# roncapat/UNIGE-TASI-path-planners

Measured on AMD Instinct MI355X. Metric: grid cells updated/sec (full plan + 100 replans), 4096^2 map, higher is better.
Workload: dtype f32

## Files before the change

### unige-tasi-path-planners_amd/csrc/ufm_control.h

```cpp
#pragma once

__global__ void k_fill(float *p, size_t n, float v) {
    for (size_t i = (size_t)blockIdx.x * blockDim.x + threadIdx.x; i < n; i += (size_t)gridDim.x * blockDim.x) p[i] = v;
}

__device__ __forceinline__ void patch_apply(const DevParams &P, int m, const uint8_t *patch, uint8_t *pmask, int x, int y, int w, int h, int e) {
    if (e >= w * h) return;
    const int i = e / w, j = e - i * w;
    uint8_t *cm = P.cost + (size_t)m * P.cstride;
    const size_t ci = (size_t)(x + i) * P.W + (y + j);
    const uint8_t nv = patch[e];
    const uint8_t ch = cm[ci] != nv;
    pmask[e] = ch;
    if (ch) { cm[ci] = nv; cost_window_store(P, m, x + i, y + j, nv); }
}
__global__ void k_patch_apply(DevParams P, int m, const uint8_t *patch, uint8_t *pmask, int x, int y, int w, int h) {
    patch_apply(P, m, patch, pmask, x, y, w, h, blockIdx.x * blockDim.x + threadIdx.x);
}
template <bool NODES>
__device__ __forceinline__ void patch_seed(const DevParams &P, int m, const uint8_t *pmask, int x, int y, int w, int h, int e) {
    const int ew = NODES ? w + 1 : w, eh = NODES ? h + 1 : h;
    bool hit = false;
    int gt = -1;
    if (e < ew * eh) {
        const int i = e / ew, j = e - i * ew;
        bool ch;
// ... 336 lines not shown
        const int cx = x - 1 + (q >> 1), cy = y - 1 + (q & 1);
        const float c = cst(cx, cy), g1 = h ? val(x, y + dy) : val(x + dx, y), g2 = val(x + dx, y + dy);
        float r; int dep;
        if constexpr (ALGO == UFM_ALGO_SG) { CellSG k; k.set(c); r = tri_sg(g1, g2, k); dep = dep_sg(g1, g2, k); }
        else {
            const float bb = h ? cst(x - 1 + (1 - (q >> 1)), cy) : cst(cx, y - 1 + (1 - (q & 1)));
            CellFD k{c, c * c, c * SQRT2F}; TriFD t; t.set(c, bb);
            r = tri_fd(g1, g2, k, t); dep = dep_fd(g1, g2, k, t);
        }
        if (r > g || r != r) {
            const float B = P.dyn->focused ? start_bound(P, m) : INFINITY;
            if (g + tile_heuristic(P, m, x / T, y / T) < B || B == INFINITY) ++n_bad; else ++n_parked;
        }
        else if (r < g) ++n_low;
        else if (dep != (b & 3)) ++n_dep;
    }
    if (n_val) atomicAdd(&out[0], n_val);
    if (n_none) atomicAdd(&out[1], n_none);
    if (n_bad) atomicAdd(&out[2], n_bad);
    if (n_dep) atomicAdd(&out[3], n_dep);
    if (n_low) atomicAdd(&out[4], n_low);
    if (n_parked) atomicAdd(&out[5], n_parked);
}
__global__ void k_cost_stats(const uint8_t *cm, size_t n, int thr, unsigned long long *out) {
    unsigned long long s = 0, c = 0;
    for (size_t i = (size_t)blockIdx.x * blockDim.x + threadIdx.x; i < n; i += (size_t)gridDim.x * blockDim.x) {
        const int v = cm[i];
        if (v < thr) { s += v; ++c; }
    }
    for (int o = 32; o > 0; o >>= 1) { s += __shfl_down(s, o); c += __shfl_down(c, o); }
    if ((threadIdx.x & 63) == 0) { atomicAdd(&out[0], s); atomicAdd(&out[1], c); }
}
__device__ __forceinline__ void finalize_tiles(const DevParams &P) {
    const int n = P.ctr->tcount;
    for (int i = blockIdx.x; i < n; i += gridDim.x) {
        const int gt = P.tlist[i];
        const size_t gidx = (size_t)gt * TT + threadIdx.x;
        const int diff = (threadIdx.x < T * T) && (P.fresh[gt] ? (P.G[gidx] != INFINITY) : (P.G[gidx] != P.Gprev[gidx]));
        const int c = __syncthreads_count(diff);
        if (threadIdx.x == 0) {
            if (c) atomicAdd(&P.ctr->expanded, (unsigned long long)c);
            P.touched[gt] = 0;
        }
    }
}
__global__ __launch_bounds__(256) void k_finalize(DevParams P, int only_if_done) {
    if (only_if_done && !P.ctr->done) return;
    const int n = P.ctr->tcount;
    const int lane = threadIdx.x & 63;
    const int wave = (blockIdx.x * blockDim.x + threadIdx.x) >> 6, nwaves = (gridDim.x * blockDim.x) >> 6;
    unsigned long long total = 0;
    for (int i = wave; i < n; i += nwaves) {
        const int gt = P.tlist[i];
        const float *g = P.G + (size_t)gt * TT, *g0 = P.Gprev + (size_t)gt * TT;
        int c = 0;
        if (P.fresh[gt]) {
#pragma unroll
            for (int e = lane; e < TT; e += 64) c += (g[e] != INFINITY) ? 1 : 0;
        } else {
#pragma unroll
            for (int e = lane; e < TT; e += 64) c += (g[e] != g0[e]) ? 1 : 0;
        }
        total += (unsigned long long)c;
        if (lane == 0) P.touched[gt] = 0;
    }
    for (int o = 32; o > 0; o >>= 1) total += __shfl_down(total, o);
    if (lane == 0 && total) atomicAdd(&P.ctr->expanded, total);
}
template <int ALGO>
__device__ void tile_bp(const DevParams &P, int gt, int thr, float *Gs, float *Cs) {
    constexpr int CROWS = is_dfm<ALGO> ? T : T + 1, COFF = is_dfm<ALGO> ? 0 : 1, CN = CROWS * CROWS;
    const int tid = threadIdx.x, w = tid >> 6, lane = tid & 63, q = lane & 3, nd = lane >> 2;
    const int m = gt / P.NTm, t = gt - m * P.NTm, tx = t / P.TY, ty = t - tx * P.TY, x0 = tx * T, y0 = ty * T;
    const float *Gt = P.G + (size_t)gt * TT, *ring = P.ring + (size_t)gt * RING;
    const uint8_t *ct = P.costT + (size_t)gt * CTS;
    for (int e = tid; e < TT; e += 256) Gs[(e / T + 1) * GP + e % T + 1] = Gt[e];
    for (int ht = tid; ht < 4 * T + 4; ht += 256) {
        int hr, hc;
        if (ht < T) { hr = -1; hc = ht; }
        else if (ht < 2 * T) { hr = T; hc = ht - T; }
        else if (ht < 3 * T) { hr = ht - 2 * T; hc = -1; }
        else if (ht < 4 * T) { hr = ht - 3 * T; hc = T; }
        else { hr = (ht & 2) ? T : -1; hc = (ht & 1) ? T : -1; }
        Gs[(hr + 1) * GP + hc + 1] = ring[ht];
    }
    for (int e = tid; e < CN; e += 256) {
        const int cr = e / CROWS, cc = e - cr * CROWS, cx = x0 + cr - COFF, cy = y0 + cc - COFF, c = ct[e];
        Cs[cr * CP + cc] = (cx < 0 || cy < 0 || cx >= P.L || cy >= P.W || c >= thr) ? INFINITY : (float)c;
    }
    __syncthreads();
    const int goal_x = P.goal[2 * m], goal_y = P.goal[2 * m + 1];
    for (int p = w; p < PT * PT; p += 4) {
        const int lx = (p / PT) * 4 + (nd >> 2), ly = (p % PT) * 4 + (nd & 3);
        QuadConsts<ALGO> C;
        C.load(Cs, lx, ly, q);
        const LaneEval le = eval_quad_w<ALGO>(Gs + (lx + 1) * GP + ly + 1, q, C);
        const float nv = quad_min(le.r);
        const int bq = quad_min_int(bp_byte<ALGO>(le, q, C, le.r == nv)), b = bp_of_key<ALGO>(bq);
        if (q == 0) P.bp[(size_t)gt * TT + lx * T + ly] = (uint8_t)((x0 + lx == goal_x && y0 + ly == goal_y) ? BP_NONE : b);
    }
    __syncthreads();
}
template <int ALGO>
__global__ __launch_bounds__(256) void k_finalize_bp(DevParams P, int only_if_done) {
    __shared__ float Gs[(T + 2) * GP];
    __shared__ float Cs[(T + 1) * CP];
    if (only_if_done && !P.ctr->done) return;
    const int n = P.ctr->tcount, thr = P.dyn->thr;
    for (int i = blockIdx.x; i < n; i += gridDim.x) tile_bp<ALGO>(P, P.tlist[i], thr, Gs, Cs);
}
__global__ __launch_bounds__(T * T) void k_replan_end(DevParams P, int kr, int kl, float margin,
                                                      DevCounters *host, unsigned int *flag, unsigned int seq) {
    __shared__ int s_m, s_done, s_last;
    kr = launch_index(P, Q_RAISE, kr);
    kl = launch_index(P, Q_LOWER, kl);
    if (seq == 0) seq = P.ctr->pubseq;
    const int done = replan_check(P, kr, kl, margin, blockIdx.x == 0, s_m, s_done);
    if (done) finalize_tiles(P);
    __threadfence();
    __syncthreads();
    if (threadIdx.x == 0) s_last = (atomicAdd(&P.ctr->fin_blocks, 1) == (int)gridDim.x - 1);
    __syncthreads();
    if (!s_last) return;
    __threadfence();
    if (threadIdx.x == 0) P.ctr->fin_blocks = 0;
    const int *src = reinterpret_cast<const int *>(P.ctr);
    int *dst = reinterpret_cast<int *>(host);
    for (int i = threadIdx.x; i < (int)(sizeof(DevCounters) / sizeof(int)); i += blockDim.x)
        dst[i] = __hip_atomic_load(&src[i], __ATOMIC_RELAXED, __HIP_MEMORY_SCOPE_AGENT);
    __threadfence_system();
    __syncthreads();
    if (threadIdx.x == 0) __hip_atomic_store(flag, seq, __ATOMIC_RELEASE, __HIP_MEMORY_SCOPE_SYSTEM);
// ... 41 lines not shown
```

### unige-tasi-path-planners_amd/csrc/ufm_defs.h

```cpp
#pragma once


#ifndef UFM_TILE
#define UFM_TILE 16
#endif
constexpr int T = UFM_TILE;
static_assert(T == 32 || T == 16, "tile edge must be 32 or 16");
constexpr int GP = T + 8;
constexpr int CP = T + 2;
constexpr int PT = T / 4;
constexpr int PR = PT / 4;
constexpr int PPW = PR * PR;
constexpr int NTHR = 1024;
#ifndef UFM_RELAX_WAVES
#define UFM_RELAX_WAVES 4
#endif
#ifndef UFM_CAUSAL_FILTER
#define UFM_CAUSAL_FILTER 1
#endif
#ifndef UFM_STEP_FILTER
#define UFM_STEP_FILTER 1
#endif
#ifndef UFM_DFM1_LAX_VISITS
#define UFM_DFM1_LAX_VISITS 64
// ... 115 lines not shown
    int npark[2];
    int nready[2];
    int rcursor[2];
    int nshort[2];
    int last_work[2];
    int fin_blocks;
    int kbase[2];
    unsigned int pubseq;
    int tcount;
    int scount;
    unsigned long long expanded;
    unsigned long long tile_visits;
    unsigned long long tile_iters;
    unsigned long long elem_evals;
    int qmin[2];
    float rbound;
    int done;
    unsigned int updated;
    int done_fail;
    unsigned long long raise_visits;
    int own_stops;
    int own_abort;
    unsigned long long own_vis0, own_vis1;
};

struct DevDyn {
    float hm;
    int thr;
    int focused;
    int pad;
};

struct DevParams {
    float *G;
    float *Gprev;
    uint8_t *bp;
    float *ring;
    float *seen;
    uint8_t *cost;
    uint8_t *costT;
    int *goal;
    int *cand;
    int *ready;
    int *hint;
    int *rank;
    int *park;
// ... 177 lines not shown
```

### unige-tasi-path-planners_amd/csrc/ufm_engine.hip

```cpp
#include <hip/hip_runtime.h>
#include <hip/hip_ext.h>

#include <chrono>
#include <climits>
#include <cmath>
#include <cstddef>
#include <cstdio>
#include <cstdlib>
#include <cstring>
#include <new>
#include <type_traits>
#include <thread>
#include <vector>

#include "../../include/ufm.h"

namespace {

#include "ufm_defs.h"
#include "ufm_ops.h"
#include "ufm_relax.h"
#include "ufm_control.h"

#include "ufm_region.h"
// ... 50 lines not shown
int ufm_debug_tiles(unsigned int *out, int n) {
    if (n > TILE_DIAG_MAX) n = TILE_DIAG_MAX;
    for (int r = 0; r < 5; ++r)
        if (hipMemcpyFromSymbol(out + (size_t)r * n, HIP_SYMBOL(g_tile), sizeof(unsigned int) * n, sizeof(unsigned int) * (size_t)r * TILE_DIAG_MAX) != hipSuccess) return UFM_ERR_HIP_BASE;
    return n;
}
int ufm_debug_wtrace(unsigned long long *out, unsigned int *counts) {
    if (hipMemcpyFromSymbol(out, HIP_SYMBOL(g_wtrace), sizeof(unsigned long long) * 16 * 256 * 2) != hipSuccess) return UFM_ERR_HIP_BASE;
    if (hipMemcpyFromSymbol(counts, HIP_SYMBOL(g_nw), sizeof(unsigned int) * 16) != hipSuccess) return UFM_ERR_HIP_BASE;
    unsigned int z[16] = {};
    hipMemcpyToSymbol(HIP_SYMBOL(g_nw), z, sizeof(z));
    return UFM_OK;
}
int ufm_debug_tdiag(unsigned long long *out, int reset) {
    if (out && hipMemcpyFromSymbol(out, HIP_SYMBOL(g_tdiag), sizeof(unsigned long long) * 64) != hipSuccess) return UFM_ERR_HIP_BASE;
    if (reset) { unsigned long long z[64] = {}; if (hipMemcpyToSymbol(HIP_SYMBOL(g_tdiag), z, sizeof(z)) != hipSuccess) return UFM_ERR_HIP_BASE; }
    return UFM_OK;
}
#endif
int ufm_debug_lmax(ufm_t *p, int32_t *out, int n) {
    if (!p || !p->e->allocated || n > LMAX) return UFM_ERR_INVALID;
    hipStreamSynchronize(p->e->stream);
    return hipMemcpy(out, p->e->P.lmax, sizeof(int) * n, hipMemcpyDeviceToHost) == hipSuccess ? UFM_OK : UFM_ERR_HIP_BASE;
}
int ufm_debug_set_tile_order(ufm_t *p, const float *a, int n) {
    if (!p || !p->e->allocated || !a || n != p->e->P.NT) return UFM_ERR_INVALID;
    hipStreamSynchronize(p->e->stream);
    if (hipMemcpy(p->e->P.dag_a, a, sizeof(float) * (size_t)n, hipMemcpyHostToDevice) != hipSuccess) return UFM_ERR_HIP_BASE;
    p->e->dag_have = true;
    return UFM_OK;
}
int ufm_tile_edge(void) { return T; }
#ifdef UFM_STRICT_FENCES
const char *ufm_version(void) { return "ufm-gfx950 0.1 (block-FIM, strict-fence checking build)"; }
#else
const char *ufm_version(void) { return T == 32 ? "ufm-gfx950 0.1 (block-FIM, tile 32)" : "ufm-gfx950 0.1 (block-FIM, tile 16)"; }
#endif

int ufm_create(ufm_t **out, int algo, int opt_lvl, int use_heuristic, int device_id) {
    if (!out) return UFM_ERR_INVALID;
    Engine *e = nullptr;
    int rc = engine_create(&e, 1, algo, opt_lvl, use_heuristic, device_id);
    if (rc != UFM_OK) return rc;
    *out = new ufm_planner{e};
    return UFM_OK;
}
// ... 298 lines not shown
```

### unige-tasi-path-planners_amd/csrc/ufm_host.h

```cpp
#pragma once

#define HIPCHK(expr)                                                      \
    do {                                                                  \
        hipError_t _e = (expr);                                           \
        if (_e != hipSuccess) return UFM_ERR_HIP_BASE - (int)_e;          \
    } while (0)

struct PatchRect { int m, x, y, w, h; };

#include "ufm_path.h"

struct MapState {
    bool initialize_search = true;
    bool goal_set = false;
    bool new_goal = false;
    bool new_start = false;
    bool have_map = false;
    bool start_set = false;
    float start_x = 0, start_y = 0, goal_x = 0, goal_y = 0;
    int goal_ex = 0, goal_ey = 0;
    bool goal_elem_valid = false;
};

struct Engine {
// ... 26 lines not shown
    int owned_waves = 0;
    int dag_mode = 0;
    bool dag_have = false;
    float dag_kappa = 0.5f;
    int dag_patience = 16;
    bool dfm_follow_info = false;
    bool use_region = true;
    int region_ahead = 2;
    int region_tiles = 6;
    int region_sweeps = 4096;
    int region_debug = 0;
    float region_band = 1.5f;
    uint32_t region_runs = 0, region_done = 0;
    uint32_t region_cont = 0, region_cont_done = 0;
    int cont_raise = 4, cont_lower = 8;
    int batch_margin = 1;
    float raise_margin = 0.25f;
    ReplanJob *h_job = nullptr;
    struct GraphSig { DevParams P; float band, delta; int max_iters, grid, follow; };
    GraphSig graph_sig{};
    std::vector<std::pair<int, hipGraphExec_t>> graphs;
    int relax_kernel(int mode, int k_arg, float rbound, int grid);
    void finalize_bp(int only_if_done) {
        if (algo == UFM_ALGO_FD) k_finalize_bp<UFM_ALGO_FD><<<2048, 256, 0, stream>>>(P, only_if_done);
        else if (algo == UFM_ALGO_SG) k_finalize_bp<UFM_ALGO_SG><<<2048, 256, 0, stream>>>(P, only_if_done);
        else if (opt_lvl >= 1) k_finalize_bp<ALGO_DFM1><<<2048, 256, 0, stream>>>(P, only_if_done);
    }
    int tail_grid = 96;
    int replan_graph(int nr, int nl, float band, hipGraphExec_t *out);
    void drop_graphs() { for (auto &g : graphs) hipGraphExecDestroy(g.second); graphs.clear(); }
    int *h_scratch = nullptr;
    int *d_scratch = nullptr;
    uint8_t *d_patch = nullptr;
    size_t d_patch_cap = 0;
    uint8_t *h_patch = nullptr;
    float *d_field = nullptr;
    size_t d_field_cap = 0;
    int32_t *d_info = nullptr;
    size_t d_info_cap = 0;
    uint8_t *d_pmask = nullptr;
    size_t d_pmask_cap = 0;
    PathJob *d_jobs = nullptr, *h_jobs = nullptr;
    float *d_path = nullptr, *h_path = nullptr;
    size_t path_cap = 0;
    std::vector<MapState> maps;
    std::vector<PatchRect> pending;
    std::vector<PatchRect> region_rects;
    int iter[2] = {0, 0};
    bool focused = true;
// ... 53 lines not shown
    int flush_lazy();
    int ensure_pmask(size_t n);
    bool region_fits(const int (*rects)[5], int nrect, int m, int *tx0, int *ntx, int *ty0, int *nty) const;
    bool track = false;
    float *trk_g = nullptr;
    uint8_t *trk_key = nullptr;
    void *trk_rec = nullptr;
    size_t trk_cap = 0;
    hipEvent_t trk_ev[2] = {nullptr, nullptr};
    float trk_scan_ms = 0.0f;
    int track_alloc();
    int track_reset(int m);
    int track_records(size_t cap);
    void track_free();
    bool lazy_region_ok() const;
};

void Engine::release() {
    if (!allocated) return;
    if (stream) hipStreamSynchronize(stream);
    track_free();
    drop_graphs();
    deferred.clear();
    std::memset(&graph_sig, 0, sizeof(graph_sig));
    void *ptrs[] = {P.G, P.Gprev, P.bp, P.ring, P.seen, P.cost, P.costT, P.goal, P.cand, P.ready, P.hint, P.rank, P.park, P.pflag, P.pprio,
                    P.queued, P.prio, P.start, P.bnd, P.dyn, P.spos, P.touched, P.fresh, P.tlist, P.sflag, P.slist, P.slist2,
                    P.mark, P.num_updated, P.consume, P.lmax, P.own_prio, P.own_lock, P.own_min, P.dag_a, P.dag_thr, P.dag_left, P.ctr, d_scratch};
    for (void *q : ptrs) if (q) hipFree(q);
    P = DevParams{};
    d_scratch = nullptr;
    allocated = false;
}

int Engine::alloc(int width, int length) {
    release();
    W = width; L = length;
    const bool nodes = algo != UFM_ALGO_DFM;
    P.W = W; P.L = L;
    P.EX = nodes ? L + 1 : L;
    P.EY = nodes ? W + 1 : W;
    P.TX = (P.EX + T - 1) / T;
    P.TY = (P.EY + T - 1) / T;
    if ((long long)P.TX * P.TY * nmaps > (long long)INT32_MAX / 4 || (long long)P.EX * P.EY > INT32_MAX) return UFM_ERR_NOMEM;
    P.NTm = P.TX * P.TY;
    P.nmaps = nmaps;
    P.NT = P.NTm * nmaps;
// ... 52 lines not shown
    dmalloc(P.dag_left, sizeof(int) * own_words());
    dmalloc(P.ctr, sizeof(DevCounters));
    dmalloc(d_scratch, sizeof(int) * (4 * nmaps + 16));
    if (rc != UFM_OK) { release(); return rc; }
    rc = [&]() -> int {
        HIPCHK(hipMemsetAsync(P.cand, 0, sizeof(int) * 6 * P.NT, stream));
        HIPCHK(hipMemsetAsync(P.park, 0, sizeof(int) * 4 * P.NT, stream));
        HIPCHK(hipMemsetAsync(P.ready, 0, sizeof(int) * P.NT, stream));
        HIPCHK(hipMemsetAsync(P.tlist, 0, sizeof(int) * P.NT, stream));
        HIPCHK(hipMemsetAsync(P.slist, 0, sizeof(int) * P.NT, stream));
        HIPCHK(hipMemsetAsync(P.slist2, 0, sizeof(int) * P.NT, stream));
        HIPCHK(hipMemsetAsync(P.rank, 0, sizeof(int) * P.NT, stream));
        HIPCHK(hipMemsetAsync(P.hint, 0, sizeof(int) * P.NT, stream));
        HIPCHK(hipMemsetAsync(P.spos, 0, sizeof(float) * 2 * nmaps, stream));
        HIPCHK(hipMemsetAsync(P.start, 0xFF, sizeof(int) * 4 * nmaps, stream));
        HIPCHK(hipMemsetAsync(P.ctr, 0, sizeof(DevCounters), stream));
        { int rq = reset_queues(); if (rq != UFM_OK) return rq; }
        HIPCHK(hipMemsetAsync(P.touched, 0, sizeof(int) * P.NT, stream));
        HIPCHK(hipMemsetAsync(P.fresh, 0, (size_t)P.NT, stream));
        HIPCHK(hipMemsetAsync(P.sflag, 0, sizeof(int) * P.NT, stream));
        HIPCHK(hipMemsetAsync(P.mark, 0, P.mstride * nmaps, stream));
        HIPCHK(hipMemsetAsync(P.num_updated, 0, sizeof(unsigned int) * nmaps, stream));
        HIPCHK(hipMemsetAsync(P.goal, 0xFF, sizeof(int) * 2 * nmaps, stream));
        k_fill<<<1024, 256, 0, stream>>>(P.G, P.gstride * nmaps, INFINITY);
        k_fill<<<1024, 256, 0, stream>>>(P.Gprev, P.gstride * nmaps, INFINITY);
        HIPCHK(hipMemsetAsync(P.bp, BP_NONE, P.gstride * nmaps, stream));
        k_fill<<<1024, 256, 0, stream>>>(P.ring, (size_t)P.NT * RING, INFINITY);
        dyn_dev = DevDyn{heur ? heuristic_multiplier : 0.0f, thr_uchar, focused ? 1 : 0, 0};
        k_set_dyn<<<1, 1, 0, stream>>>(P.dyn, dyn_dev);
        HIPCHK(hipGetLastError());
        return UFM_OK;
    }();
    if (rc != UFM_OK) { release(); return rc; }
    if (track) { rc = track_alloc(); if (rc != UFM_OK) { release(); return rc; } }
    pending.clear();
    for (auto &ms : maps) { ms.have_map = false; ms.initialize_search = true; }
    return UFM_OK;
}

int Engine::reset_queues() {
    HIPCHK(hipMemsetAsync(P.queued, 0, sizeof(int) * 4 * P.NT, stream));
    HIPCHK(hipMemsetAsync(P.prio, 0xFF, sizeof(unsigned long long) * 4 * P.NT, stream));
    HIPCHK(hipMemsetAsync(P.pflag, 0, sizeof(int) * 2 * P.NT, stream));
    k_fill<<<64, 256, 0, stream>>>(reinterpret_cast<float *>(P.pprio), (size_t)2 * P.NT, INFINITY);
    k_fill<<<64, 256, 0, stream>>>(reinterpret_cast<float *>(P.own_prio), own_words(), INFINITY);
    HIPCHK(hipMemsetAsync(P.own_lock, 0, sizeof(int) * own_words(), stream));
    k_fill<<<2, 256, 0, stream>>>(reinterpret_cast<float *>(P.own_min), (size_t)OWN_NW, INFINITY);
    static_assert(offsetof(DevCounters, cnt) == 0, "queue state leads the counter block");
    HIPCHK(hipMemsetAsync(P.ctr, 0, offsetof(DevCounters, kbase), stream));
    k_fill<<<1, 64, 0, stream>>>(reinterpret_cast<float *>(&P.ctr->lmin[0][0]), (size_t)6, INFINITY);
    last_active = 1;
    iter[0] = iter[1] = 0;
    return UFM_OK;
}
int Engine::read_bounds(float *bmax) {
    k_start_bound<<<(nmaps + 63) / 64, 64, 0, stream>>>(P);
    HIPCHK(hipMemcpyAsync(h_bnd, P.bnd, sizeof(float) * nmaps, hipMemcpyDeviceToHost, stream));
    HIPCHK(hipStreamSynchronize(stream));
    float b = 0.0f;
    for (int m = 0; m < nmaps; ++m) b = std::fmax(b, h_bnd[m]);
    *bmax = b;
    return UFM_OK;
}

__global__ void k_publish(const DevCounters *src, DevCounters *dst, unsigned int *flag, unsigned int seq) {
    const int *s = reinterpret_cast<const int *>(src);
    int *d = reinterpret_cast<int *>(dst);
    for (int i = threadIdx.x; i < (int)(sizeof(DevCounters) / sizeof(int)); i += blockDim.x) d[i] = s[i];
    __threadfence_system();
    __syncthreads();
    if (threadIdx.x == 0) __hip_atomic_store(flag, seq, __ATOMIC_RELEASE, __HIP_MEMORY_SCOPE_SYSTEM);
}
int Engine::fetch_counters() {
// ... 375 lines not shown
    }
    const DevDyn dyn_now{heur ? heuristic_multiplier : 0.0f, thr_uchar, focused ? 1 : 0, 0};
    bool dyn_pending = std::memcmp(&dyn_now, &dyn_dev, sizeof(DevDyn)) != 0;
    auto flush_dyn = [&]() {
        if (!dyn_pending) return;
        k_set_dyn<<<1, 1, 0, stream>>>(P.dyn, dyn_now);
        dyn_dev = dyn_now; dyn_pending = false;
    };

    int n_init = 0, n_upd = 0;
    int *consume = h_scratch, *init_tiles = h_scratch + nmaps, *goals = h_scratch + 2 * nmaps;
    {
        bool all_init = true;
        for (int m = 0; m < nmaps; ++m) all_init = all_init && (maps[m].initialize_search || maps[m].new_goal);
        if (all_init) { int rc = reset_queues(); if (rc != UFM_OK) return rc; }
    }
    for (int m = 0; m < nmaps; ++m) {
        MapState &ms = maps[m];
        consume[m] = 0;
        if (ms.initialize_search || ms.new_goal) {
            consume[m] = 1;
            goals[2 * m] = ms.goal_elem_valid ? ms.goal_ex : -1;
            goals[2 * m + 1] = ms.goal_elem_valid ? ms.goal_ey : -1;
            k_fill<<<1024, 256, 0, stream>>>(P.G + (size_t)m * P.gstride, P.gstride, INFINITY);
            HIPCHK(hipMemsetAsync(P.bp + (size_t)m * P.gstride, BP_NONE, P.gstride, stream));
            k_fill<<<256, 256, 0, stream>>>(P.ring + (size_t)m * P.NTm * RING, (size_t)P.NTm * RING, INFINITY);
            if (ms.goal_elem_valid) init_tiles[n_init++] = m * P.NTm + (ms.goal_ex / T) * P.TY + (ms.goal_ey / T);
            else ++n_init;
        } else if (ms.new_start) {
            ms.new_start = false;
            consume[m] = 1;
            ++n_upd;
        }
    }
    for (int m = 0; m < nmaps; ++m) {
        MapState &ms = maps[m];
        if (ms.initialize_search || ms.new_goal)
            HIPCHK(hipMemcpyAsync(P.goal + 2 * m, goals + 2 * m, 2 * sizeof(int), hipMemcpyHostToDevice, stream));
    }
    ReplanBegin rb{};
    bool fused = single && fuse_control && spin_wait && n_init == 0 && n_upd > 0 && !pending.empty() && pending.size() <= 4;
    if (fused)
        for (const PatchRect &r : pending) fused = fused && consume[r.m] && (r.w + 1) * (r.h + 1) <= 65 * 65;
    {
        int *st_el = h_scratch + 5 * nmaps + 4;
        float *sp = reinterpret_cast<float *>(h_scratch + 9 * nmaps + 8);
        for (int m = 0; m < nmaps; ++m) {
            const MapState &ms = maps[m];
            for (int i = 0; i < 4; ++i) st_el[4 * m + i] = -1;
            sp[2 * m] = sp[2 * m + 1] = 0.0f;
            if (!ms.start_set) continue;
            const int cx = (int)(start_cell_floor ? std::floor(ms.start_x) : std::roundf(ms.start_x)), cy = (int)(start_cell_floor ? std::floor(ms.start_y) : std::roundf(ms.start_y));
            sp[2 * m] = (algo == UFM_ALGO_DFM) ? (float)cx : ms.start_x;
            sp[2 * m + 1] = (algo == UFM_ALGO_DFM) ? (float)cy : ms.start_y;
            const int ncorner = (algo == UFM_ALGO_DFM) ? 1 : 4;
            for (int i = 0; i < ncorner; ++i) {
                const int ex = cx + (i & 1), ey = cy + (i >> 1);
// ... 291 lines not shown
                owned_left = h_ctr->cnt[Q_LOWER][iter[Q_LOWER] % 3];
            }
            int rc = owned_left == 0 ? UFM_OK : run_phase(MODE_LOWER, INFINITY, &ll, &st.kernel_ms, &st.timed_launches);
            if (rc != UFM_OK) return rc;
            st.launches += ll;
            bool again = false;
            if (focused && do_raise) {
                float bnew = 0.0f;
                rc = read_bounds(&bnew);
                if (rc != UFM_OK) return rc;
                k_queue_min<<<1, 1024, 0, stream>>>(P, Q_RAISE, iter[Q_RAISE]);
                rc = fetch_counters();
                if (rc != UFM_OK) return rc;
                float qm;
                std::memcpy(&qm, &h_ctr->qmin[Q_RAISE], sizeof(float));
                if (qm < bnew) { again = true; rbound = std::fmax(bnew, rbound) + band; }
            }
            const auto tc = std::chrono::steady_clock::now();
            u_acc += std::chrono::duration<double, std::milli>(tb - ta).count();
            p_acc += std::chrono::duration<double, std::milli>(tc - tb).count();
            if (!again) break;
        }
        const auto td = std::chrono::steady_clock::now();
        finalize_bp(0);
        k_finalize<<<2048, 256, 0, stream>>>(P, 0);
        { int rc = fetch_counters(); if (rc != UFM_OK) return rc; }
        st.expanded = h_ctr->expanded;
        st.tile_visits = h_ctr->tile_visits;
        st.tile_iters = h_ctr->tile_iters;
        st.elem_evals = h_ctr->elem_evals;
        st.raise_tile_visits = h_ctr->raise_visits;
        if (st.resident_launches) {
            st.resident_tile_visits = h_ctr->own_vis1 - h_ctr->own_vis0;
            st.resident_stops = (uint32_t)h_ctr->own_stops;
            if (own_timed) HIPCHK(hipEventElapsedTime(&st.resident_kernel_ms, own_ev[0], own_ev[1]));
        }
        if (profiling) {
            std::vector<int> lm(LMAX);
            HIPCHK(hipMemcpy(lm.data(), P.lmax, sizeof(int) * LMAX, hipMemcpyDeviceToHost));
            for (int v : lm) st.crit_sweeps += (uint64_t)v;
        }
        p_acc += std::chrono::duration<double, std::milli>(std::chrono::steady_clock::now() - td).count();
    } else if (fast_done) {
        st.expanded = h_ctr->expanded;
        st.tile_visits = h_ctr->tile_visits;
        st.tile_iters = h_ctr->tile_iters;
        st.elem_evals = h_ctr->elem_evals;
        st.raise_tile_visits = h_ctr->raise_visits;
        const double dt = std::chrono::duration<double, std::milli>(std::chrono::steady_clock::now() - t_seed).count();
        u_acc += 0.5 * dt;
        p_acc += 0.5 * dt;
    } else {
        HIPCHK(hipStreamSynchronize(stream));
    }
    for (int m = 0; m < nmaps; ++m) maps[m].new_goal = maps[m].initialize_search = false;
    st.updated = updated;
    st.queued_lower = (uint32_t)(h_ctr->cnt[Q_LOWER][iter[Q_LOWER] % 3] + h_ctr->npark[Q_LOWER]);
    st.queued_raise = (uint32_t)(h_ctr->cnt[Q_RAISE][iter[Q_RAISE] % 3] + h_ctr->npark[Q_RAISE]);
    st.graphs_instantiated = graphs_made;
    st.region_replans = region_runs; st.region_replans_done = region_done;
    st.u_ms = (float)u_acc;
    st.p_ms = (float)p_acc;
    last = st;
    if (out) *out = st;
// ... 80 lines not shown
    if (e->h_lazy) hipHostFree(e->h_lazy);
    e->drop_graphs();
    if (e->h_ctr) hipHostFree(e->h_ctr);
    for (int i = 0; i < 2; ++i) if (e->h_pipe_ctr[i]) hipHostFree(e->h_pipe_ctr[i]);
    if (e->h_job) hipHostFree(e->h_job);
    if (e->h_scratch) hipHostFree(e->h_scratch);
    if (e->h_bnd) hipHostFree(e->h_bnd);
    if (e->stream) hipStreamDestroy(e->stream);
    delete e;
    return UFM_OK;
}

int engine_set_map(Engine *e, int m, const uint8_t *src, bool on_device, int width, int length) {
    if (!e || !src || m < 0 || m >= e->nmaps || width <= 0 || length <= 0) return UFM_ERR_INVALID;
    HIPCHK(hipSetDevice(e->device));
    if (e->allocated) { int rc = e->flush_deferred(); if (rc != UFM_OK) return rc; }
    if (!e->allocated || width != e->W || length != e->L) {
        bool others = false;
        for (int k = 0; k < e->nmaps; ++k) if (k != m && e->maps[k].have_map) others = true;
        if (e->allocated && others) return UFM_ERR_INVALID;
        int rc = e->alloc(width, length);
        if (rc != UFM_OK) return rc;
    }
    HIPCHK(hipMemcpyAsync(e->P.cost + (size_t)m * e->P.cstride, src, (size_t)width * length,
                          on_device ? hipMemcpyDeviceToDevice : hipMemcpyHostToDevice, e->stream));
    k_cost_windows<<<2048, 256, 0, e->stream>>>(e->P, m);
    {
        unsigned long long *d_acc = reinterpret_cast<unsigned long long *>(e->d_scratch);
        HIPCHK(hipMemsetAsync(d_acc, 0, 2 * sizeof(unsigned long long), e->stream));
        k_cost_stats<<<512, 256, 0, e->stream>>>(e->P.cost + (size_t)m * e->P.cstride, (size_t)width * length, e->thr_uchar, d_acc);
        unsigned long long *h_acc = reinterpret_cast<unsigned long long *>(e->h_scratch);
        HIPCHK(hipMemcpyAsync(h_acc, d_acc, 2 * sizeof(unsigned long long), hipMemcpyDeviceToHost, e->stream));
        HIPCHK(hipStreamSynchronize(e->stream));
        if (h_acc[1] > 0) e->mean_cost = (float)((double)h_acc[0] / (double)h_acc[1]);
    }
    if (e->track) { int rc = e->track_reset(m); if (rc != UFM_OK) return rc; }
    e->maps[m].have_map = true;
    MapState &ms = e->maps[m];
    if (ms.goal_set) ms.goal_elem_valid = ms.goal_ex >= 0 && ms.goal_ey >= 0 && ms.goal_ex < e->P.EX && ms.goal_ey < e->P.EY;
    return UFM_OK;
}

int engine_patch(Engine *e, int m, const uint8_t *src, bool on_device, int x, int y, int w, int h) {
    if (!e || !src) return UFM_ERR_INVALID;
    HIPCHK(hipSetDevice(e->device));
    if (on_device) return e->patch(m, src, x, y, w, h, true);
    if (w <= 0 || h <= 0) return UFM_ERR_INVALID;
    {
        bool taken = false;
        const int rc = e->patch_lazy(m, src, x, y, w, h, &taken);
        if (rc != UFM_OK || taken) return rc;
    }
    const size_t n = (size_t)w * h;
// ... 164 lines not shown
```

Measured before the change: 566.5 million.

## Batch fills, fuse set_map stats with window build, wave-per-tile finalize

Replaces the many separate fill kernels and memsets with one table-driven fill kernel that writes 16-byte stores. Fuses the cost copy, the cost statistics and the tile window construction into a single k_set_map kernel. Fuses the finalize expanded-count into the backpointer kernel, which now assigns one wave per tile and uses wave-local LDS waits instead of block barriers. Also moves the lmax sum for profiling onto the device. These cut launch overhead and redundant passes over memory, at the cost of more complex code and more LDS per block.

```diff
diff --git a/unige-tasi-path-planners_amd/csrc/ufm_control.h b/unige-tasi-path-planners_amd/csrc/ufm_control.h
--- a/unige-tasi-path-planners_amd/csrc/ufm_control.h
+++ b/unige-tasi-path-planners_amd/csrc/ufm_control.h
@@ -2,6 +2,23 @@
 
 __global__ void k_fill(float *p, size_t n, float v) {
     for (size_t i = (size_t)blockIdx.x * blockDim.x + threadIdx.x; i < n; i += (size_t)gridDim.x * blockDim.x) p[i] = v;
+}
+
+constexpr int FILL_MAX = 24;
+struct FillTable { int n; struct { void *p; size_t bytes; unsigned int pat; } e[FILL_MAX]; };
+__global__ __launch_bounds__(256) void k_fill_table(FillTable t) {
+    const size_t gtid = (size_t)blockIdx.x * blockDim.x + threadIdx.x, gsz = (size_t)gridDim.x * blockDim.x;
+    for (int k = 0; k < t.n; ++k) {
+        unsigned int *w = static_cast<unsigned int *>(t.e[k].p);
+        const unsigned int pat = t.e[k].pat;
+        const size_t nw = t.e[k].bytes / 4;
+        const size_t lead = ((16 - (reinterpret_cast<uintptr_t>(w) & 15)) & 15) / 4, head = lead < nw ? lead : nw, nv = (nw - head) / 4, tail0 = head + nv * 4;
+        uint4 *v = reinterpret_cast<uint4 *>(w + head);
+        const uint4 pv = make_uint4(pat, pat, pat, pat);
+        for (size_t i = gtid; i < nv; i += gsz) v[i] = pv;
+        if (gtid < head) w[gtid] = pat;
+        if (gtid < nw - tail0) w[tail0 + gtid] = pat;
+    }
 }
 
 __device__ __forceinline__ void patch_apply(const DevParams &P, int m, const uint8_t *patch, uint8_t *pmask, int x, int y, int w, int h, int e) {
@@ -384,15 +401,90 @@
     if (n_low) atomicAdd(&out[4], n_low);
     if (n_parked) atomicAdd(&out[5], n_parked);
 }
-__global__ void k_cost_stats(const uint8_t *cm, size_t n, int thr, unsigned long long *out) {
-    unsigned long long s = 0, c = 0;
-    for (size_t i = (size_t)blockIdx.x * blockDim.x + threadIdx.x; i < n; i += (size_t)gridDim.x * blockDim.x) {
-        const int v = cm[i];
-        if (v < thr) { s += v; ++c; }
-    }
-    for (int o = 32; o > 0; o >>= 1) { s += __shfl_down(s, o); c += __shfl_down(c, o); }
-    if ((threadIdx.x & 63) == 0) { atomicAdd(&out[0], s); atomicAdd(&out[1], c); }
-}
+constexpr int SM_TILES = 16;
+constexpr int SM_CH = SM_TILES * T / 16;
+constexpr int SM_PITCH = SM_TILES * T + 16;
+template <bool CELLS>
+__global__ __launch_bounds__(256) void k_set_map(DevParams P, int m, const uint8_t *src, int thr, unsigned long long *out) {
+    constexpr int CROWS = CELLS ? T : T + 1, OFF = CELLS ? 0 : 1, CN = CROWS * CROWS, NCH = (CN + 15) / 16;
+    static_assert(NCH * 16 <= CTS, "the 16-byte stores stay inside a window record");
+    __shared__ __attribute__((aligned(16))) uint8_t s[(T + 1) * SM_PITCH];
+    const int nstrips = (P.TY + SM_TILES - 1) / SM_TILES;
+    const int tx = blockIdx.x / nstrips, ty0 = (blockIdx.x - tx * nstrips) * SM_TILES, x0 = tx * T, y0 = ty0 * T;
+    uint8_t *cm = P.cost + (size_t)m * P.cstride;
+    const bool copy = src != cm;
+    const bool vec = ((reinterpret_cast<uintptr_t>(src) | reinterpret_cast<uintptr_t>(cm) | (uintptr_t)P.W) & 15) == 0;
+    unsigned int sum = 0, cnt = 0;
+    for (int task = threadIdx.x; task < (T + 1) * (SM_CH + 1); task += blockDim.x) {
+        const int r = task / (SM_CH + 1), k = task - r * (SM_CH + 1) - 1;
+        const int cx = x0 - 1 + r;
+        const bool rowin = cx >= 0 && cx < P.L && !(CELLS && r == 0), own = r > 0;
+        if (k < 0) {
+            const int cy = y0 - 1;
+            s[r * SM_PITCH + 15] = (rowin && !CELLS && cy >= 0 && cy < P.W) ? src[(size_t)cx * P.W + cy] : (uint8_t)255;
+            continue;
+        }
+        const int cy = y0 + 16 * k;
+        unsigned int w[4] = {~0u, ~0u, ~0u, ~0u};
+        if (rowin && cy < P.W) {
+            const size_t a = (size_t)cx * P.W + cy;
+            if (vec) {
+                const uint4 v = *reinterpret_cast<const uint4 *>(src + a);
+                if (own && copy) *reinterpret_cast<uint4 *>(cm + a) = v;
+                w[0] = v.x; w[1] = v.y; w[2] = v.z; w[3] = v.w;
+                if (own) {
+#pragma unroll
+                    for (int j = 0; j < 16; ++j) {
+                        const int b = (int)((w[j >> 2] >> (8 * (j & 3))) & 255u);
+                        if (b < thr) { sum += (unsigned int)b; ++cnt; }
+                    }
+                }
+            } else {
+#pragma unroll
+                for (int j = 0; j < 16; ++j) {
+                    if (cy + j >= P.W) continue;
+                    const int b = src[a + j];
+                    w[j >> 2] = (w[j >> 2] & ~(255u << (8 * (j & 3)))) | ((unsigned int)b << (8 * (j & 3)));
+                    if (!own) continue;
+                    if (copy) cm[a + j] = (uint8_t)b;
+                    if (b < thr) { sum += (unsigned int)b; ++cnt; }
+                }
+            }
+        }
+        *reinterpret_cast<uint4 *>(&s[r * SM_PITCH + 16 + 16 * k]) = make_uint4(w[0], w[1], w[2], w[3]);
+    }
+    for (int o = 32; o > 0; o >>= 1) { sum += __shfl_down(sum, o); cnt += __shfl_down(cnt, o); }
+    if ((threadIdx.x & 63) == 0 && cnt) { atomicAdd(&out[0], (unsigned long long)sum); atomicAdd(&out[1], (unsigned long long)cnt); }
+    __syncthreads();
+    for (int task = threadIdx.x; task < SM_TILES * NCH; task += blockDim.x) {
+        const int j = task / NCH, q = task - j * NCH, ty = ty0 + j;
+        if (ty >= P.TY) continue;
+        unsigned int w[4] = {0u, 0u, 0u, 0u};
+#pragma unroll
+        for (int b = 0; b < 16; ++b) {
+            const int e = 16 * q + b;
+            if (e >= CN) continue;
+            const int cr = e / CROWS, cc = e - cr * CROWS;
+            w[b >> 2] |= (unsigned int)s[(cr + 1 - OFF) * SM_PITCH + 16 - OFF + T * j + cc] << (8 * (b & 3));
+        }
+        *reinterpret_cast<uint4 *>(P.costT + ((size_t)m * P.NTm + (size_t)tx * P.TY + ty) * CTS + 16 * q) = make_uint4(w[0], w[1], w[2], w[3]);
+    }
+}
+__device__ void sum_lmax(const DevParams &P) {
+    __shared__ unsigned long long s_part[16];
+    unsigned long long v = 0;
+    for (int i = threadIdx.x; i < LMAX; i += blockDim.x) v += (unsigned long long)P.lmax[i];
+    for (int o = 32; o > 0; o >>= 1) v += __shfl_down(v, o);
+    if ((threadIdx.x & 63) == 0) s_part[threadIdx.x >> 6] = v;
+    __syncthreads();
+    if (threadIdx.x == 0) {
+        unsigned long long t = 0;
+        for (int i = 0; i < (int)(blockDim.x + 63) / 64; ++i) t += s_part[i];
+        P.ctr->crit_sweeps = t;
+    }
+    __syncthreads();
+}
+__global__ __launch_bounds__(1024) void k_sum_lmax(DevParams P) { sum_lmax(P); }
 __device__ __forceinline__ void finalize_tiles(const DevParams &P) {
     const int n = P.ctr->tcount;
     for (int i = blockIdx.x; i < n; i += gridDim.x) {
@@ -429,30 +521,57 @@
     for (int o = 32; o > 0; o >>= 1) total += __shfl_down(total, o);
     if (lane == 0 && total) atomicAdd(&P.ctr->expanded, total);
 }
-template <int ALGO>
-__device__ void tile_bp(const DevParams &P, int gt, int thr, float *Gs, float *Cs) {
+__device__ __forceinline__ void wave_lds_sync() { asm volatile("s_waitcnt lgkmcnt(0)" ::: "memory"); }
+template <int ALGO, bool COUNT>
+__device__ __forceinline__ int tile_bp(const DevParams &P, int gt, int thr, float *Gs, float *Cs) {
     constexpr int CROWS = is_dfm<ALGO> ? T : T + 1, COFF = is_dfm<ALGO> ? 0 : 1, CN = CROWS * CROWS;
-    const int tid = threadIdx.x, w = tid >> 6, lane = tid & 63, q = lane & 3, nd = lane >> 2;
+    static_assert((CN + 15) / 16 * 16 <= CTS && (4 * T + 4) % 4 == 0 && 4 * T + 4 <= RING, "the 16-byte loads stay inside the records");
+    const int lane = threadIdx.x & 63, q = lane & 3, nd = lane >> 2;
     const int m = gt / P.NTm, t = gt - m * P.NTm, tx = t / P.TY, ty = t - tx * P.TY, x0 = tx * T, y0 = ty * T;
-    const float *Gt = P.G + (size_t)gt * TT, *ring = P.ring + (size_t)gt * RING;
-    const uint8_t *ct = P.costT + (size_t)gt * CTS;
-    for (int e = tid; e < TT; e += 256) Gs[(e / T + 1) * GP + e % T + 1] = Gt[e];
-    for (int ht = tid; ht < 4 * T + 4; ht += 256) {
-        int hr, hc;
-        if (ht < T) { hr = -1; hc = ht; }
-        else if (ht < 2 * T) { hr = T; hc = ht - T; }
-        else if (ht < 3 * T) { hr = ht - 2 * T; hc = -1; }
-        else if (ht < 4 * T) { hr = ht - 3 * T; hc = T; }
-        else { hr = (ht & 2) ? T : -1; hc = (ht & 1) ? T : -1; }
-        Gs[(hr + 1) * GP + hc + 1] = ring[ht];
-    }
-    for (int e = tid; e < CN; e += 256) {
-        const int cr = e / CROWS, cc = e - cr * CROWS, cx = x0 + cr - COFF, cy = y0 + cc - COFF, c = ct[e];
-        Cs[cr * CP + cc] = (cx < 0 || cy < 0 || cx >= P.L || cy >= P.W || c >= thr) ? INFINITY : (float)c;
-    }
-    __syncthreads();
+    const float4 *Gt = reinterpret_cast<const float4 *>(P.G + (size_t)gt * TT), *G0 = reinterpret_cast<const float4 *>(P.Gprev + (size_t)gt * TT);
+    const float4 *ring = reinterpret_cast<const float4 *>(P.ring + (size_t)gt * RING);
+    const uint4 *ct = reinterpret_cast<const uint4 *>(P.costT + (size_t)gt * CTS);
+    const bool fresh = COUNT && P.fresh[gt];
+    int changed = 0;
+#pragma unroll
+    for (int v = lane; v < TT / 4; v += 64) {
+        const float4 g = Gt[v];
+        float *d = Gs + ((4 * v) / T + 1) * GP + (4 * v) % T + 1;
+        d[0] = g.x; d[1] = g.y; d[2] = g.z; d[3] = g.w;
+        if constexpr (COUNT) {
+            if (fresh) changed += (g.x != INFINITY) + (g.y != INFINITY) + (g.z != INFINITY) + (g.w != INFINITY);
+            else { const float4 g0 = G0[v]; changed += (g.x != g0.x) + (g.y != g0.y) + (g.z != g0.z) + (g.w != g0.w); }
+        }
+    }
+    for (int v = lane; v < (4 * T + 4) / 4; v += 64) {
+        const float4 r4 = ring[v];
+        const float rv[4] = {r4.x, r4.y, r4.z, r4.w};
+#pragma unroll
+        for (int k = 0; k < 4; ++k) {
+            const int ht = 4 * v + k;
+            int hr, hc;
+            if (ht < T) { hr = -1; hc = ht; }
+            else if (ht < 2 * T) { hr = T; hc = ht - T; }
+            else if (ht < 3 * T) { hr = ht - 2 * T; hc = -1; }
+            else if (ht < 4 * T) { hr = ht - 3 * T; hc = T; }
+            else { hr = (ht & 2) ? T : -1; hc = (ht & 1) ? T : -1; }
+            Gs[(hr + 1) * GP + hc + 1] = rv[k];
+        }
+    }
+    for (int v = lane; v < (CN + 15) / 16; v += 64) {
+        const uint4 c4 = ct[v];
+        const unsigned int cw[4] = {c4.x, c4.y, c4.z, c4.w};
+#pragma unroll
+        for (int k = 0; k < 16; ++k) {
+            const int e = 16 * v + k;
+            if (e >= CN) continue;
+            const int cr = e / CROWS, cc = e - cr * CROWS, cx = x0 + cr - COFF, cy = y0 + cc - COFF, c = (int)((cw[k >> 2] >> (8 * (k & 3))) & 255u);
+            Cs[cr * CP + cc] = (cx < 0 || cy < 0 || cx >= P.L || cy >= P.W || c >= thr) ? INFINITY : (float)c;
+        }
+    }
+    wave_lds_sync();
     const int goal_x = P.goal[2 * m], goal_y = P.goal[2 * m + 1];
-    for (int p = w; p < PT * PT; p += 4) {
+    for (int p = 0; p < PT * PT; ++p) {
         const int lx = (p / PT) * 4 + (nd >> 2), ly = (p % PT) * 4 + (nd & 3);
         QuadConsts<ALGO> C;
         C.load(Cs, lx, ly, q);
@@ -461,15 +580,23 @@
         const int bq = quad_min_int(bp_byte<ALGO>(le, q, C, le.r == nv)), b = bp_of_key<ALGO>(bq);
         if (q == 0) P.bp[(size_t)gt * TT + lx * T + ly] = (uint8_t)((x0 + lx == goal_x && y0 + ly == goal_y) ? BP_NONE : b);
     }
-    __syncthreads();
-}
-template <int ALGO>
+    wave_lds_sync();
+    if (COUNT && lane == 0) P.touched[gt] = 0;
+    return changed;
+}
+template <int ALGO, bool COUNT>
 __global__ __launch_bounds__(256) void k_finalize_bp(DevParams P, int only_if_done) {
-    __shared__ float Gs[(T + 2) * GP];
-    __shared__ float Cs[(T + 1) * CP];
+    __shared__ float Gs[4][(T + 2) * GP];
+    __shared__ float Cs[4][(T + 1) * CP];
     if (only_if_done && !P.ctr->done) return;
     const int n = P.ctr->tcount, thr = P.dyn->thr;
-    for (int i = blockIdx.x; i < n; i += gridDim.x) tile_bp<ALGO>(P, P.tlist[i], thr, Gs, Cs);
+    const int w = threadIdx.x >> 6, wave = blockIdx.x * 4 + w, nwaves = gridDim.x * 4;
+    unsigned long long total = 0;
+    for (int i = wave; i < n; i += nwaves) total += (unsigned long long)tile_bp<ALGO, COUNT>(P, P.tlist[i], thr, Gs[w], Cs[w]);
+    if constexpr (COUNT) {
+        for (int o = 32; o > 0; o >>= 1) total += __shfl_down(total, o);
+        if ((threadIdx.x & 63) == 0 && total) atomicAdd(&P.ctr->expanded, total);
+    }
 }
 __global__ __launch_bounds__(T * T) void k_replan_end(DevParams P, int kr, int kl, float margin,
                                                       DevCounters *host, unsigned int *flag, unsigned int seq) {
diff --git a/unige-tasi-path-planners_amd/csrc/ufm_defs.h b/unige-tasi-path-planners_amd/csrc/ufm_defs.h
--- a/unige-tasi-path-planners_amd/csrc/ufm_defs.h
+++ b/unige-tasi-path-planners_amd/csrc/ufm_defs.h
@@ -161,6 +161,7 @@
     int own_stops;
     int own_abort;
     unsigned long long own_vis0, own_vis1;
+    unsigned long long crit_sweeps;
 };
 
 struct DevDyn {
diff --git a/unige-tasi-path-planners_amd/csrc/ufm_engine.hip b/unige-tasi-path-planners_amd/csrc/ufm_engine.hip
--- a/unige-tasi-path-planners_amd/csrc/ufm_engine.hip
+++ b/unige-tasi-path-planners_amd/csrc/ufm_engine.hip
@@ -96,6 +96,13 @@
     if (!p || !p->e->allocated || n > LMAX) return UFM_ERR_INVALID;
     hipStreamSynchronize(p->e->stream);
     return hipMemcpy(out, p->e->P.lmax, sizeof(int) * n, hipMemcpyDeviceToHost) == hipSuccess ? UFM_OK : UFM_ERR_HIP_BASE;
+}
+static float engine_band(const Engine *e) { return e->delta_abs >= 0.0f ? e->delta_abs : e->delta_scale * T * e->mean_cost; }
+int ufm_debug_band(ufm_t *p, float *out) { if (!p || !out) return UFM_ERR_INVALID; *out = engine_band(p->e); return UFM_OK; }
+int ufm_batch_debug_band(ufm_batch_t *b, int i, float *out) {
+    if (!b || !out || i < 0 || i >= b->n_maps) return UFM_ERR_INVALID;
+    *out = engine_band(b->shards[i / b->per]);
+    return UFM_OK;
 }
 int ufm_debug_set_tile_order(ufm_t *p, const float *a, int n) {
     if (!p || !p->e->allocated || !a || n != p->e->P.NT) return UFM_ERR_INVALID;
diff --git a/unige-tasi-path-planners_amd/csrc/ufm_host.h b/unige-tasi-path-planners_amd/csrc/ufm_host.h
--- a/unige-tasi-path-planners_amd/csrc/ufm_host.h
+++ b/unige-tasi-path-planners_amd/csrc/ufm_host.h
@@ -72,9 +72,27 @@
     std::vector<std::pair<int, hipGraphExec_t>> graphs;
     int relax_kernel(int mode, int k_arg, float rbound, int grid);
     void finalize_bp(int only_if_done) {
-        if (algo == UFM_ALGO_FD) k_finalize_bp<UFM_ALGO_FD><<<2048, 256, 0, stream>>>(P, only_if_done);
-        else if (algo == UFM_ALGO_SG) k_finalize_bp<UFM_ALGO_SG><<<2048, 256, 0, stream>>>(P, only_if_done);
-        else if (opt_lvl >= 1) k_finalize_bp<ALGO_DFM1><<<2048, 256, 0, stream>>>(P, only_if_done);
+        if (algo == UFM_ALGO_FD) k_finalize_bp<UFM_ALGO_FD, false><<<2048, 256, 0, stream>>>(P, only_if_done);
+        else if (algo == UFM_ALGO_SG) k_finalize_bp<UFM_ALGO_SG, false><<<2048, 256, 0, stream>>>(P, only_if_done);
+        else if (opt_lvl >= 1) k_finalize_bp<ALGO_DFM1, false><<<2048, 256, 0, stream>>>(P, only_if_done);
+    }
+    void finalize_plan() {
+        if (algo == UFM_ALGO_FD) k_finalize_bp<UFM_ALGO_FD, true><<<2048, 256, 0, stream>>>(P, 0);
+        else if (algo == UFM_ALGO_SG) k_finalize_bp<UFM_ALGO_SG, true><<<2048, 256, 0, stream>>>(P, 0);
+        else if (opt_lvl >= 1) k_finalize_bp<ALGO_DFM1, true><<<2048, 256, 0, stream>>>(P, 0);
+        else k_finalize<<<2048, 256, 0, stream>>>(P, 0);
+    }
+    FillTable fills{};
+    void fill(void *p, size_t bytes, unsigned int pat) {
+        if (!bytes) return;
+        if (fills.n == FILL_MAX) flush_fills();
+        fills.e[fills.n].p = p; fills.e[fills.n].bytes = bytes; fills.e[fills.n].pat = pat;
+        ++fills.n;
+    }
+    void flush_fills() {
+        if (!fills.n) return;
+        k_fill_table<<<1024, 256, 0, stream>>>(fills);
+        fills.n = 0;
     }
     int tail_grid = 96;
     int replan_graph(int nr, int nl, float band, hipGraphExec_t *out);
@@ -174,6 +192,7 @@
     track_free();
     drop_graphs();
     deferred.clear();
+    fills.n = 0;
     std::memset(&graph_sig, 0, sizeof(graph_sig));
     void *ptrs[] = {P.G, P.Gprev, P.bp, P.ring, P.seen, P.cost, P.costT, P.goal, P.cand, P.ready, P.hint, P.rank, P.park, P.pflag, P.pprio,
                     P.queued, P.prio, P.start, P.bnd, P.dyn, P.spos, P.touched, P.fresh, P.tlist, P.sflag, P.slist, P.slist2,
@@ -272,10 +291,11 @@
         HIPCHK(hipMemsetAsync(P.mark, 0, P.mstride * nmaps, stream));
         HIPCHK(hipMemsetAsync(P.num_updated, 0, sizeof(unsigned int) * nmaps, stream));
         HIPCHK(hipMemsetAsync(P.goal, 0xFF, sizeof(int) * 2 * nmaps, stream));
-        k_fill<<<1024, 256, 0, stream>>>(P.G, P.gstride * nmaps, INFINITY);
-        k_fill<<<1024, 256, 0, stream>>>(P.Gprev, P.gstride * nmaps, INFINITY);
-        HIPCHK(hipMemsetAsync(P.bp, BP_NONE, P.gstride * nmaps, stream));
-        k_fill<<<1024, 256, 0, stream>>>(P.ring, (size_t)P.NT * RING, INFINITY);
+        fill(P.G, gbytes, (unsigned int)INFBITS);
+        fill(P.Gprev, gbytes, (unsigned int)INFBITS);
+        fill(P.bp, P.gstride * nmaps, BP_NONE * 0x01010101u);
+        fill(P.ring, (size_t)P.NT * RING * sizeof(float), (unsigned int)INFBITS);
+        flush_fills();
         dyn_dev = DevDyn{heur ? heuristic_multiplier : 0.0f, thr_uchar, focused ? 1 : 0, 0};
         k_set_dyn<<<1, 1, 0, stream>>>(P.dyn, dyn_dev);
         HIPCHK(hipGetLastError());
@@ -289,16 +309,18 @@
 }
 
 int Engine::reset_queues() {
-    HIPCHK(hipMemsetAsync(P.queued, 0, sizeof(int) * 4 * P.NT, stream));
-    HIPCHK(hipMemsetAsync(P.prio, 0xFF, sizeof(unsigned long long) * 4 * P.NT, stream));
-    HIPCHK(hipMemsetAsync(P.pflag, 0, sizeof(int) * 2 * P.NT, stream));
-    k_fill<<<64, 256, 0, stream>>>(reinterpret_cast<float *>(P.pprio), (size_t)2 * P.NT, INFINITY);
-    k_fill<<<64, 256, 0, stream>>>(reinterpret_cast<float *>(P.own_prio), own_words(), INFINITY);
-    HIPCHK(hipMemsetAsync(P.own_lock, 0, sizeof(int) * own_words(), stream));
-    k_fill<<<2, 256, 0, stream>>>(reinterpret_cast<float *>(P.own_min), (size_t)OWN_NW, INFINITY);
-    static_assert(offsetof(DevCounters, cnt) == 0, "queue state leads the counter block");
-    HIPCHK(hipMemsetAsync(P.ctr, 0, offsetof(DevCounters, kbase), stream));
-    k_fill<<<1, 64, 0, stream>>>(reinterpret_cast<float *>(&P.ctr->lmin[0][0]), (size_t)6, INFINITY);
+    fill(P.queued, sizeof(int) * 4 * P.NT, 0u);
+    fill(P.prio, sizeof(unsigned long long) * 4 * P.NT, ~0u);
+    fill(P.pflag, sizeof(int) * 2 * P.NT, 0u);
+    fill(P.pprio, sizeof(int) * 2 * P.NT, (unsigned int)INFBITS);
+    fill(P.own_prio, sizeof(int) * own_words(), (unsigned int)INFBITS);
+    fill(P.own_lock, sizeof(int) * own_words(), 0u);
+    fill(P.own_min, sizeof(int) * OWN_NW, (unsigned int)INFBITS);
+    static_assert(offsetof(DevCounters, cnt) == 0 && offsetof(DevCounters, lmin) < offsetof(DevCounters, npark), "queue state leads the counter block");
+    char *c = reinterpret_cast<char *>(P.ctr);
+    fill(c, offsetof(DevCounters, lmin), 0u);
+    fill(c + offsetof(DevCounters, lmin), sizeof(P.ctr->lmin), (unsigned int)INFBITS);
+    fill(c + offsetof(DevCounters, npark), offsetof(DevCounters, kbase) - offsetof(DevCounters, npark), 0u);
     last_active = 1;
     iter[0] = iter[1] = 0;
     return UFM_OK;
@@ -720,9 +742,9 @@
             consume[m] = 1;
             goals[2 * m] = ms.goal_elem_valid ? ms.goal_ex : -1;
             goals[2 * m + 1] = ms.goal_elem_valid ? ms.goal_ey : -1;
-            k_fill<<<1024, 256, 0, stream>>>(P.G + (size_t)m * P.gstride, P.gstride, INFINITY);
-            HIPCHK(hipMemsetAsync(P.bp + (size_t)m * P.gstride, BP_NONE, P.gstride, stream));
-            k_fill<<<256, 256, 0, stream>>>(P.ring + (size_t)m * P.NTm * RING, (size_t)P.NTm * RING, INFINITY);
+            fill(P.G + (size_t)m * P.gstride, P.gstride * sizeof(float), (unsigned int)INFBITS);
+            fill(P.bp + (size_t)m * P.gstride, P.gstride, BP_NONE * 0x01010101u);
+            fill(P.ring + (size_t)m * P.NTm * RING, (size_t)P.NTm * RING * sizeof(float), (unsigned int)INFBITS);
             if (ms.goal_elem_valid) init_tiles[n_init++] = m * P.NTm + (ms.goal_ex / T) * P.TY + (ms.goal_ey / T);
             else ++n_init;
         } else if (ms.new_start) {
@@ -731,6 +753,8 @@
             ++n_upd;
         }
     }
+    flush_fills();
+    HIPCHK(hipGetLastError());
     for (int m = 0; m < nmaps; ++m) {
         MapState &ms = maps[m];
         if (ms.initialize_search || ms.new_goal)
@@ -1068,8 +1092,8 @@
             if (!again) break;
         }
         const auto td = std::chrono::steady_clock::now();
-        finalize_bp(0);
-        k_finalize<<<2048, 256, 0, stream>>>(P, 0);
+        finalize_plan();
+        if (profiling) k_sum_lmax<<<1, 1024, 0, stream>>>(P);
         { int rc = fetch_counters(); if (rc != UFM_OK) return rc; }
         st.expanded = h_ctr->expanded;
         st.tile_visits = h_ctr->tile_visits;
@@ -1081,11 +1105,7 @@
             st.resident_stops = (uint32_t)h_ctr->own_stops;
             if (own_timed) HIPCHK(hipEventElapsedTime(&st.resident_kernel_ms, own_ev[0], own_ev[1]));
         }
-        if (profiling) {
-            std::vector<int> lm(LMAX);
-            HIPCHK(hipMemcpy(lm.data(), P.lmax, sizeof(int) * LMAX, hipMemcpyDeviceToHost));
-            for (int v : lm) st.crit_sweeps += (uint64_t)v;
-        }
+        if (profiling) st.crit_sweeps = h_ctr->crit_sweeps;
         p_acc += std::chrono::duration<double, std::milli>(std::chrono::steady_clock::now() - td).count();
     } else if (fast_done) {
         st.expanded = h_ctr->expanded;
@@ -1212,13 +1232,15 @@
         int rc = e->alloc(width, length);
         if (rc != UFM_OK) return rc;
     }
-    HIPCHK(hipMemcpyAsync(e->P.cost + (size_t)m * e->P.cstride, src, (size_t)width * length,
-                          on_device ? hipMemcpyDeviceToDevice : hipMemcpyHostToDevice, e->stream));
-    k_cost_windows<<<2048, 256, 0, e->stream>>>(e->P, m);
     {
+        uint8_t *cm = e->P.cost + (size_t)m * e->P.cstride;
+        if (!on_device) { HIPCHK(hipMemcpyAsync(cm, src, (size_t)width * length, hipMemcpyHostToDevice, e->stream)); src = cm; }
         unsigned long long *d_acc = reinterpret_cast<unsigned long long *>(e->d_scratch);
         HIPCHK(hipMemsetAsync(d_acc, 0, 2 * sizeof(unsigned long long), e->stream));
-        k_cost_stats<<<512, 256, 0, e->stream>>>(e->P.cost + (size_t)m * e->P.cstride, (size_t)width * length, e->thr_uchar, d_acc);
+        const unsigned int nblk = (unsigned int)e->P.TX * (unsigned int)((e->P.TY + SM_TILES - 1) / SM_TILES);
+        if (e->P.cells) k_set_map<true><<<nblk, 256, 0, e->stream>>>(e->P, m, src, e->thr_uchar, d_acc);
+        else k_set_map<false><<<nblk, 256, 0, e->stream>>>(e->P, m, src, e->thr_uchar, d_acc);
+        HIPCHK(hipGetLastError());
         unsigned long long *h_acc = reinterpret_cast<unsigned long long *>(e->h_scratch);
         HIPCHK(hipMemcpyAsync(h_acc, d_acc, 2 * sizeof(unsigned long long), hipMemcpyDeviceToHost, e->stream));
         HIPCHK(hipStreamSynchronize(e->stream));
```

New measurement: 562.2 million. About the same (-0.8%).
